# Thefefe/orbit

Hardware: AMD Instinct MI355X
Metric: meshlets_culled_per_sec (higher is better)
Workload: dtype f32

## Files before the change

### bindings/rust/orbit_hip.rs

```rust
#![allow(non_camel_case_types, dead_code)]
use std::ffi::{c_char, c_void};

#[repr(C)]
pub struct OrbitCtx { _private: [u8; 0] }
#[repr(C)]
pub struct OrbitMeshletStream { _private: [u8; 0] }

#[repr(C)] #[derive(Clone, Copy, Default)]
pub struct OrbitCaps {
    pub max_entities: u32, pub max_dispatches: u32, pub max_draws: u32, pub max_lights: u32,
    pub max_clusters: u32, pub dispatch_size: u32, pub max_views: u32, pub validate_streams: u32, pub cull_path: u32,
    pub arith_profile: u32,
}

#[repr(C)]
pub struct OrbitClusterFrame {
    pub push: *const c_void, pub info: *const c_void, pub depth: *const f32, pub lights: *const c_void,
    pub tile_depth_slice_mask: *mut u32, pub depth_bounds: *mut c_void, pub unique_cluster_buffer: *mut c_void,
    pub light_index_buffer: *mut c_void, pub cluster_offset_image: *mut u32,
    pub index_capacity: u32, pub light_index_capacity: u32,
}
#[repr(C)]
pub struct OrbitFrameLate {
    pub pyramids: *const c_void, pub late_views: *const c_void, pub cascade_views: *const c_void,
// ... 202 lines not shown
    pub fn orbit_meshlet_stream_set_materials(ctx: *mut OrbitCtx, ms: *mut OrbitMeshletStream, material_buffer: *const c_void,
                                              material_count: u32, stream: *mut c_void) -> i32;
    pub fn orbit_meshlet_stream_validate(ctx: *mut OrbitCtx, ms: *mut OrbitMeshletStream, meshlet_buffer: *const c_void,
                                         material_buffer: *const c_void, stream: *mut c_void) -> i32;
    pub fn orbit_meshlet_stream_destroy(ms: *mut OrbitMeshletStream) -> i32;
    pub fn orbit_meshlet_stream_update_meshes(ctx: *mut OrbitCtx, ms: *mut OrbitMeshletStream, mesh_info_buffer: *const c_void,
                                              first_mesh: u32, count: u32, stream: *mut c_void) -> i32;
    pub fn orbit_ctx_mesh_side_culls(ctx: *const OrbitCtx) -> u64;
    pub fn orbit_ctx_bind_meshlet_stream(ctx: *mut OrbitCtx, ms: *mut OrbitMeshletStream) -> i32;
    pub fn orbit_ctx_fused_culls(ctx: *const OrbitCtx) -> u64;
    pub fn orbit_frame_late(ctx: *mut OrbitCtx, frame: *const OrbitFrameLate, stream: *mut c_void) -> i32;
    pub fn orbit_ctx_meshlet_stream_culls(ctx: *const OrbitCtx) -> u64;
    pub fn orbit_ctx_meshlet_class_culls(ctx: *const OrbitCtx) -> u64;
    pub fn orbit_ctx_block_culls(ctx: *const OrbitCtx) -> u64;
    pub fn orbit_ctx_set_block_cull(ctx: *mut OrbitCtx, enable: u32) -> i32;
    pub fn orbit_meshlet_stream_block_bounds(ctx: *mut OrbitCtx, ms: *mut OrbitMeshletStream, first_block: u64, count: u64,
                                             out: *mut c_void, stream: *mut c_void) -> i32;
    pub fn orbit_p2p_alloc(ctx: *mut OrbitCtx, bytes: u64, out_ptr: *mut *mut c_void, out_handle: *mut [u8; 64]) -> i32;
    pub fn orbit_p2p_free(ctx: *mut OrbitCtx, ptr: *mut c_void) -> i32;
    pub fn orbit_p2p_open(ctx: *mut OrbitCtx, handle: *const [u8; 64], out_peer_ptr: *mut *mut c_void) -> i32;
    pub fn orbit_p2p_close(ctx: *mut OrbitCtx, peer_ptr: *mut c_void) -> i32;
    pub fn orbit_meshlet_cull_records_and_commands(ctx: *mut OrbitCtx, cull_info: *const c_void,
                                                   bufs: *const OrbitMeshletCullBufs, record_buffer: *mut c_void,
                                                   record_capacity: u32, stream: *mut c_void) -> i32;
    pub fn orbit_exchange_list(ctx: *mut OrbitCtx, local_list: *const c_void, rank: u32, world: u32,
                               out_buffers: *const *mut c_void, ctrl_buffers: *const *mut c_void, out_capacity: u32,
                               header_bytes: u32, stride: u32, stream: *mut c_void) -> i32;
    pub fn orbit_cull_shard(ctx: *mut OrbitCtx, cull_info: *const c_void, entity_bufs: *const OrbitEntityCullBufs,
                            draw_first: u32, draw_count: u32, meshlet_bufs: *const OrbitMeshletCullBufs,
                            record_buffer: *mut c_void, record_capacity: u32, with_commands: u32,
// ... 37 lines not shown
```

### include/orbit_abi_ext.h

```cpp
#ifndef ORBIT_ABI_EXT_H
#define ORBIT_ABI_EXT_H

#include "orbit_abi.h"

#ifdef __cplusplus
extern "C" {
#endif

#define ORBIT_VISIBLE_HEADER 8u
typedef struct OrbitVisibleRecord {
    uint32_t entity_index;
    uint32_t meshlet_offset;
    uint32_t mask;
} OrbitVisibleRecord;
ORBIT_STATIC_ASSERT(sizeof(OrbitVisibleRecord) == 12, "visible record is 12 B");

int32_t orbit_meshlet_task_cull(OrbitCtx *ctx, const OrbitGpuCullInfo *cull_info,
                                const OrbitMeshletCullBufs *bufs,
                                OrbitMeshTaskRecord *task_records, void *stream);

typedef struct OrbitCullView {
    const OrbitGpuCullInfo *cull_info;
    OrbitEntityCullBufs entity;
    OrbitMeshletCullBufs meshlet;
// ... 10 lines not shown
int32_t orbit_meshlet_stream_update(OrbitCtx *ctx, OrbitMeshletStream *ms, const void *meshlet_buffer,
                                    uint64_t first, uint64_t count, void *stream);
int32_t orbit_meshlet_stream_set_materials(OrbitCtx *ctx, OrbitMeshletStream *ms, const void *material_buffer,
                                           uint32_t material_count, void *stream);
int32_t orbit_meshlet_stream_validate(OrbitCtx *ctx, OrbitMeshletStream *ms, const void *meshlet_buffer,
                                      const void *material_buffer, void *stream);
int32_t orbit_meshlet_stream_update_meshes(OrbitCtx *ctx, OrbitMeshletStream *ms, const void *mesh_info_buffer,
                                           uint32_t first_mesh, uint32_t count, void *stream);
uint64_t orbit_ctx_mesh_side_culls(const OrbitCtx *ctx);
int32_t orbit_meshlet_stream_destroy(OrbitMeshletStream *ms);
int32_t orbit_ctx_bind_meshlet_stream(OrbitCtx *ctx, OrbitMeshletStream *ms);
uint64_t orbit_ctx_meshlet_stream_culls(const OrbitCtx *ctx);
uint64_t orbit_ctx_meshlet_class_culls(const OrbitCtx *ctx);
uint64_t orbit_ctx_block_culls(const OrbitCtx *ctx);
int32_t orbit_ctx_set_block_cull(OrbitCtx *ctx, uint32_t enable);
int32_t orbit_meshlet_stream_block_bounds(OrbitCtx *ctx, OrbitMeshletStream *ms, uint64_t first_block, uint64_t count,
                                          void *out, void *stream);

typedef struct OrbitDepthReduceItem {
    const float *depth;
    uint32_t screen_width, screen_height;
    uint32_t depth_row_pitch;
    uint32_t _pad;
    float *pyramid;
    const OrbitDepthPyramidLevel *levels;
} OrbitDepthReduceItem;
ORBIT_STATIC_ASSERT(sizeof(OrbitDepthReduceItem) == 40, "depth-reduce item is 40 B");
#define ORBIT_MAX_PYRAMID_BATCH 8
int32_t orbit_depth_reduce_multi(OrbitCtx *ctx, const OrbitDepthReduceItem *items, uint32_t count, void *stream);

// ... 268 lines not shown
```

### orbit_amd/_lib.py

```python
import ctypes as C
import os

_HERE = os.path.dirname(os.path.abspath(__file__))
LIB_PATH = os.path.join(_HERE, "liborbit_cull.so")

OK, E_INVALID, E_PLANES, E_CAPACITY, E_HIP, E_NO_DEVICE, E_TIMEOUT, E_MISSING, E_COMM, E_RANGE, E_STALE = (
    0, -1, -2, -3, -4, -5, -6, -7, -8, -9, -10)
ERROR_NAMES = {
    E_INVALID: "ORBIT_E_INVALID", E_PLANES: "ORBIT_E_PLANES", E_CAPACITY: "ORBIT_E_CAPACITY", E_HIP: "ORBIT_E_HIP",
    E_NO_DEVICE: "ORBIT_E_NO_DEVICE", E_TIMEOUT: "ORBIT_E_TIMEOUT", E_MISSING: "ORBIT_E_MISSING",
    E_COMM: "ORBIT_E_COMM", E_RANGE: "ORBIT_E_RANGE", E_STALE: "ORBIT_E_STALE",
}

MAX_PYRAMID_MIPS = 16


class OrbitError(RuntimeError):
    def __init__(self, code, message):
        super().__init__(f"{ERROR_NAMES.get(code, code)}: {message}")
        self.code = code


class Caps(C.Structure):
    _fields_ = [("max_entities", C.c_uint32), ("max_dispatches", C.c_uint32), ("max_draws", C.c_uint32),
# ... 144 lines not shown
    "orbit_p2p_open": (C.c_int32, [C.c_void_p, C.c_void_p, C.POINTER(C.c_void_p)]),
    "orbit_p2p_close": (C.c_int32, [C.c_void_p, C.c_void_p]),
    "orbit_meshlet_stream_create": (C.c_int32, [C.c_void_p, C.c_uint64, C.c_uint64, C.POINTER(C.c_void_p)]),
    "orbit_meshlet_stream_update": (C.c_int32, [C.c_void_p, C.c_void_p, C.c_void_p, C.c_uint64, C.c_uint64,
                                                C.c_void_p]),
    "orbit_meshlet_stream_set_materials": (C.c_int32, [C.c_void_p, C.c_void_p, C.c_void_p, C.c_uint32, C.c_void_p]),
    "orbit_meshlet_stream_validate": (C.c_int32, [C.c_void_p, C.c_void_p, C.c_void_p, C.c_void_p, C.c_void_p]),
    "orbit_meshlet_stream_destroy": (C.c_int32, [C.c_void_p]),
    "orbit_meshlet_stream_update_meshes": (C.c_int32, [C.c_void_p, C.c_void_p, C.c_void_p, C.c_uint32, C.c_uint32, C.c_void_p]),
    "orbit_ctx_mesh_side_culls": (C.c_uint64, [C.c_void_p]),
    "orbit_ctx_bind_meshlet_stream": (C.c_int32, [C.c_void_p, C.c_void_p]),
    "orbit_ctx_meshlet_stream_culls": (C.c_uint64, [C.c_void_p]),
    "orbit_ctx_meshlet_class_culls": (C.c_uint64, [C.c_void_p]),
    "orbit_ctx_block_culls": (C.c_uint64, [C.c_void_p]),
    "orbit_ctx_set_block_cull": (C.c_int32, [C.c_void_p, C.c_uint32]),
    "orbit_meshlet_stream_block_bounds": (C.c_int32, [C.c_void_p, C.c_void_p, C.c_uint64, C.c_uint64, C.c_void_p,
                                                      C.c_void_p]),
    "orbit_cull_shard": (C.c_int32, [C.c_void_p, C.c_void_p, C.POINTER(EntityCullBufs), C.c_uint32, C.c_uint32,
                                     C.POINTER(MeshletCullBufs), C.c_void_p, C.c_uint32, C.c_uint32, C.c_void_p]),
    "orbit_ctx_shard_culls": (C.c_uint64, [C.c_void_p]),
    "orbit_allgather_list": (C.c_int32, [C.c_void_p, C.c_void_p, C.c_uint32, C.c_uint32, C.c_void_p, C.c_uint32,
                                         C.c_void_p, C.c_void_p, C.c_uint32, C.c_uint32, C.c_uint32, C.c_void_p]),
    "orbit_compact_segments": (C.c_int32, [C.c_void_p, C.c_void_p, C.c_uint32, C.c_uint32, C.c_void_p, C.c_uint32,
                                           C.c_uint32, C.c_uint32, C.c_void_p]),
    "orbit_scene_update_entities": (C.c_int32, [C.c_void_p, C.c_void_p, C.c_void_p, C.c_uint32, C.c_void_p, C.c_uint32,
                                                C.c_void_p]),
    "orbit_scene_update": (C.c_int32, [C.c_void_p, C.POINTER(SceneUpdate), C.c_void_p]),
    "orbit_cull_stats": (C.c_int32, [C.c_void_p, C.c_void_p, C.POINTER(EntityCullBufs), C.c_uint32,
                                     C.POINTER(MeshletCullBufs), C.c_void_p, C.c_void_p]),
    "orbit_cluster_stats": (C.c_int32, [C.c_void_p, C.c_void_p, C.c_void_p, C.c_void_p, C.c_void_p, C.c_void_p,
# ... 49 lines not shown
```

### orbit_amd/csrc/abi_ctx.hip

```cpp
#include <cstdarg>
#include <cstdio>
#include <cstdlib>

#include "abi_internal.h"

thread_local char g_err[512] = "no error";

int32_t fail(OrbitCtx *ctx, int32_t code, const char *fmt, ...) {
    char buf[512];
    va_list ap;
    va_start(ap, fmt);
    vsnprintf(buf, sizeof(buf), fmt, ap);
    va_end(ap);
    snprintf(g_err, sizeof(g_err), "%s", buf);
    if (ctx) snprintf(ctx->err, sizeof(ctx->err), "%s", buf);
    return code;
}

namespace {

size_t layout_arena(OrbitCtx *ctx, uintptr_t base, uint64_t md32) {
    const OrbitCaps &caps = ctx->caps;
    const size_t ent = align_up((size_t)caps.max_entities, 256);
    const size_t mtiles = ((size_t)md32 + kTileRecords - 1) / kTileRecords + 1;
// ... 155 lines not shown
    if (!ctx) return ORBIT_OK;
    (void)hipSetDevice(ctx->device);
    (void)hipDeviceSynchronize();
    for (hipEvent_t ev : ctx->prof_events) (void)hipEventDestroy(ev);
    for (hipEvent_t ev : ctx->side_event)
        if (ev) (void)hipEventDestroy(ev);
    for (hipStream_t st : ctx->side_stream)
        if (st) (void)hipStreamDestroy(st);
    for (OrbitCtx *child : ctx->view_ctx) (void)orbit_ctx_destroy(child);
    if (ctx->meshlet_stream) ctx->meshlet_stream->bindings.fetch_sub(1);
    if (ctx->arena) (void)hipFree(ctx->arena);
    delete ctx;
    return ORBIT_OK;
}

int32_t orbit_ctx_status(OrbitCtx *ctx, void *stream, int32_t sync) {
    if (!ctx) return fail(nullptr, ORBIT_E_INVALID, "ctx is NULL");
    std::lock_guard<std::mutex> lock(ctx->mu);
    hipStream_t s = (hipStream_t)stream;
    if (sync) {
        hipError_t e = hipStreamSynchronize(s);
        if (e != hipSuccess) return hip_fail(ctx, e, "hipStreamSynchronize");
    }
    int32_t v = 0;
    hipError_t e = hipMemcpy(&v, ctx->status, 4, hipMemcpyDeviceToHost);
    if (e != hipSuccess) return hip_fail(ctx, e, "hipMemcpy(status)");
    for (OrbitCtx *child : ctx->view_ctx) {
        int32_t cv = 0;
        e = hipMemcpy(&cv, child->status, 4, hipMemcpyDeviceToHost);
        if (e != hipSuccess) return hip_fail(ctx, e, "hipMemcpy(status)");
// ... 124 lines not shown
```

### orbit_amd/csrc/abi_cull.hip

```cpp
#include "abi_internal.h"

namespace {

int32_t check_cull_info(OrbitCtx *ctx, const OrbitGpuCullInfo *ci) {
    if (!ci) return fail(ctx, ORBIT_E_INVALID, "cull_info is NULL");
    if (ci->cull_plane_count > ORBIT_MAX_CULL_PLANES)
        return fail(ctx, ORBIT_E_PLANES, "cull_plane_count %u > %d", ci->cull_plane_count, ORBIT_MAX_CULL_PLANES);
    if (ci->projection_type > 1) return fail(ctx, ORBIT_E_INVALID, "projection_type %u", ci->projection_type);
    if (ci->occlusion_pass > 2) return fail(ctx, ORBIT_E_INVALID, "occlusion_pass %u", ci->occlusion_pass);
    return ORBIT_OK;
}

MeshSideView mesh_side_for(OrbitMeshletStream *ms, const void *mesh_info_buffer, bool count = true) {
    if (!ms) return MeshSideView{nullptr, 0u};
    std::lock_guard<std::mutex> lock(ms->mu);
    if (ms->mesh_side == nullptr || ms->mesh_source != mesh_info_buffer || ms->mesh_hi == 0u) return MeshSideView{nullptr, 0u};
    if (count) ms->mesh_side_culls++;
    return MeshSideView{ms->mesh_side, ms->mesh_hi};
}

PyramidView make_pyramid_view(const float *texels, const uint32_t size[2],
                              const OrbitDepthPyramidLevel *levels = nullptr) {
    PyramidView v;
    v.texels = texels;
// ... 210 lines not shown
                          const MeshletCullOut &out, void *stream) {
    if (!ctx) return fail(nullptr, ORBIT_E_INVALID, "ctx is NULL");
    std::lock_guard<std::mutex> lock(ctx->mu);
    const hipStream_t s = (hipStream_t)stream;
    MeshletCullParams p;
    hipEvent_t ev0, ev1;
    int32_t rc = meshlet_cull_params(ctx, ctx, ci, b, out, p);
    if (rc == ORBIT_OK) rc = profile_pair(ctx, ev0, ev1);
    if (rc == ORBIT_OK && ci->occlusion_pass != 1) rc = validate_stream(ctx, p, s);
    if (rc) return rc;
    hipError_t e = hipSuccess;
    if (ctx->rec_shift > 5u) e = launch_split_records(split_params_for(ctx, ctx, b), s);
    if (e != hipSuccess) return hip_fail(ctx, e, "launch split_records");
    const bool blocks = ctx->block_cull && out.kind == MeshletCullOut::kCommands && p.ms.sphere != nullptr &&
                        p.ms.cls0 != nullptr && ci->occlusion_pass == 0u && ci->projection_type == 0u && p.arith == 0u;
    e = launch_meshlet_cull(p, ctx->num_cus, s, ev0, ev1, blocks ? stream_block_bounds(ctx->meshlet_stream) : nullptr);
    if (e != hipSuccess) return hip_fail(ctx, e, "launch meshlet_cull");
    count_stream_cull(ctx, p);
    if (blocks) ctx->block_culls++;
    return ORBIT_OK;
}

FusedCullParams fused_params(const EntityCullParams &ep, const MeshletCullParams &mp, const OrbitCtx *scratch,
                             uint32_t chunks) {
    FusedCullParams f{};
    f.m = mp;
    f.entity_draw_buffer = ep.entity_draw_buffer;
    f.mesh_infos = ep.mesh_infos;
    f.mesh_side = ep.mesh_side;
    f.visibility = ep.visibility;
    f.e_pyr = ep.pyr;
// ... 250 lines not shown
```

### orbit_amd/csrc/abi_internal.h

```cpp
#pragma once
#include <hip/hip_runtime.h>

#include <atomic>
#include <cstdint>
#include <cstring>
#include <mutex>
#include <new>
#include <vector>

#include "block_pretest.h"
#include "kernels.h"

using namespace orbit;

#pragma GCC visibility push(hidden)

struct OrbitMeshletStream {
    int device = 0;
    uint64_t first = 0, capacity = 0;
    uint4 *sphere = nullptr;
    uint32_t *cone = nullptr;
    uint16_t *mat = nullptr;
    uint32_t *cmd = nullptr;
    uint16_t *cnt = nullptr;
// ... 54 lines not shown
    uint32_t scan_patience = 256;
    unsigned long long *debug_cycles = nullptr;
    void *zero_page = nullptr;
    uint32_t profiling = 0;
    uint32_t prof_calls = 0;
    std::vector<hipEvent_t> prof_events;
    size_t prof_used = 0;
    std::vector<OrbitCtx *> view_ctx;
    hipStream_t side_stream[2] = {nullptr, nullptr};
    hipEvent_t side_event[3] = {nullptr, nullptr, nullptr};
    OrbitMeshletStream *meshlet_stream = nullptr;
    uint64_t stream_culls = 0;
    uint64_t class_culls = 0;
    uint64_t block_culls = 0;
    bool block_cull = true;
    char err[512] = {0};
};

constexpr uint32_t kExpandBlocks = 65536;

constexpr uint32_t kMeshBoundsSlots = 1024;

extern thread_local char g_err[512];

int32_t fail(OrbitCtx *ctx, int32_t code, const char *fmt, ...);

inline int32_t hip_fail(OrbitCtx *ctx, hipError_t e, const char *what) {
    return fail(ctx, ORBIT_E_HIP, "%s: %s", what, hipGetErrorString(e));
}

// ... 66 lines not shown
```

### orbit_amd/csrc/kernels.h

```cpp
#pragma once
#include <hip/hip_runtime.h>
#include <stdint.h>
#include <type_traits>

#include "../../include/orbit_abi_ext.h"
#include "orbit_device.h"

namespace orbit {

struct BlockBound;

constexpr uint32_t kTileRecords = 16;
constexpr uint32_t kTileRows = 8;
constexpr uint32_t kTicketPools = 8;
constexpr uint32_t kTicketStride = 64;
constexpr uint32_t kEmitTicketPools = 16;
constexpr uint32_t kListGroups = 32;
constexpr uint32_t kListSyncStride = 32;
constexpr uint32_t kListSyncWords = (kListGroups + 1) * kListSyncStride;

struct Payload {
    uint32_t y, z, w;
};

// ... 198 lines not shown
struct ViewGroup;
#if !ORBIT_CONTRACT
hipError_t launch_entity_cull_contracted(const EntityCullParams &p, uint32_t entity_draw_count, uint32_t num_cus, hipStream_t s);
hipError_t launch_entity_cull_views_contracted(const EntityCullViews &all, uint32_t n, uint32_t max_entity_draw_count,
                                               uint32_t num_cus, hipStream_t s);
hipError_t launch_meshlet_eval_contracted(const MeshletCullParams &p, uint32_t num_cus, hipStream_t s);
hipError_t launch_meshlet_eval_views_contracted(const MeshletCullViews &all, const ViewGroup &g, uint32_t m, uint32_t pass,
                                                bool ortho, int src, uint32_t max_tiles, uint32_t num_cus, hipStream_t s);
hipError_t launch_shard_cull_contracted(const FusedCullParams &f, uint32_t num_cus, hipStream_t s);
hipError_t launch_cull_fused_views_contracted(const FusedCullViews &all, const uint32_t *entity_draw_counts, uint32_t n,
                                              uint32_t num_cus, hipStream_t s);
#endif
hipError_t launch_entity_cull_views(const EntityCullViews &all, uint32_t n, uint32_t max_entity_draw_count,
                                    uint32_t num_cus, hipStream_t s);
hipError_t launch_meshlet_cull(const MeshletCullParams &p, uint32_t num_cus, hipStream_t s,
                               hipEvent_t ev0 = nullptr, hipEvent_t ev1 = nullptr, const BlockBound *blk = nullptr);
struct MeshletCullViews {
    MeshletCullParams v[ORBIT_MAX_CULL_VIEWS];
};
hipError_t launch_meshlet_cull_views(const MeshletCullViews &all, uint32_t n, uint32_t num_cus, hipStream_t s);
struct ViewGroup {
    uint8_t idx[ORBIT_MAX_CULL_VIEWS];
};
hipError_t launch_meshlet_eval(const MeshletCullParams &p, uint32_t num_cus, hipStream_t s);
hipError_t launch_meshlet_eval_blocks(const MeshletCullParams &p, const BlockBound *blk, dim3 grid, hipStream_t s);
uint32_t meshlet_eval_blocks_grid(uint32_t max_tiles, uint32_t num_cus);
hipError_t launch_meshlet_eval_views(const MeshletCullViews &all, const ViewGroup &g, uint32_t m, uint32_t pass,
                                     bool ortho, int src, uint32_t max_tiles, uint32_t num_cus, hipStream_t s);
hipError_t launch_meshlet_emit(const MeshletCullParams &p, bool stream, uint32_t num_cus, hipStream_t s);
hipError_t launch_meshlet_emit_views(const MeshletCullViews &all, const ViewGroup &g, uint32_t m, uint32_t n, bool stream,
                                     uint32_t max_tiles_all, uint32_t num_cus, hipStream_t s);
// ... 111 lines not shown
```

### orbit_amd/csrc/meshlet_cull.hip

```cpp
#include "kernels.h"

namespace orbit {

uint32_t max_dispatch_capacity() {
    const uint64_t cap = (uint64_t)kEmitChunkTable * kScanChunk * kTileRecords;
    return cap > 0xFFFFFFFFull ? 0xFFFFFFFFu : (uint32_t)cap;
}

namespace {

hipError_t scan_and_emit(const MeshletCullParams &p, uint32_t max_tiles, uint32_t num_cus, hipStream_t s) {
    const bool stream = p.ci.occlusion_pass != 1 && p.ms.sphere != nullptr;
    if (!stream) {
        const hipError_t e = launch_scan_chunks(p.tile_counts, p.tile_base, reinterpret_cast<const uint32_t *>(p.dispatch_buffer),
                                                kTileRecords, max_tiles, p.chunk_sums, s, p.tickets, kTicketPools * kTicketStride);
        if (e != hipSuccess) return e;
    }
    return launch_meshlet_emit(p, stream, num_cus, s);
}

}

hipError_t launch_meshlet_scan_emit(const MeshletCullParams &p, uint32_t num_cus, hipStream_t s) {
    const uint32_t max_tiles = (p.dispatch_capacity + kTileRecords - 1) / kTileRecords;
    if ((max_tiles + kScanChunk - 1) / kScanChunk > kEmitChunkTable) return hipErrorInvalidValue;
    return scan_and_emit(p, max_tiles, num_cus, s);
}

hipError_t launch_meshlet_cull(const MeshletCullParams &p, uint32_t num_cus, hipStream_t s, hipEvent_t ev0,
                               hipEvent_t ev1, const BlockBound *blk) {
    const uint32_t max_tiles = (p.dispatch_capacity + kTileRecords - 1) / kTileRecords;
    if ((max_tiles + kScanChunk - 1) / kScanChunk > kEmitChunkTable) return hipErrorInvalidValue;
    hipError_t e;
    if (ev0 && (e = hipEventRecord(ev0, s)) != hipSuccess) return e;
    if (blk != nullptr) {
        if (p.ci.occlusion_pass != 0u || p.ci.projection_type != 0u || p.arith != 0u || p.ms.cls0 == nullptr ||
            p.visible_list != 0u || p.task_records != nullptr)
            return hipErrorInvalidValue;
        e = launch_meshlet_eval_blocks(p, blk, dim3(meshlet_eval_blocks_grid(max_tiles, num_cus)), s);
    } else {
        e = launch_meshlet_eval(p, num_cus, s);
    }
    if (e != hipSuccess) return e;
    if (ev1 && (e = hipEventRecord(ev1, s)) != hipSuccess) return e;
    if (p.task_records) return launch_task_records(p, s);
    if (p.visible_list == 2u) {
        if (p.also_commands == nullptr) return hipSuccess;
        MeshletCullParams c = p;
        c.visible_list = 0u;
        c.draw_buffer = p.also_commands;
        c.draw_capacity = p.also_commands_capacity;
        return scan_and_emit(c, max_tiles, num_cus, s);
    }
    return scan_and_emit(p, max_tiles, num_cus, s);
// ... 56 lines not shown
```

### orbit_amd/csrc/meshlet_eval_blocks.hip

```cpp
#include "block_pretest.h"
#include "meshlet_common.h"

namespace orbit {

namespace {

constexpr int kBkWaves = 4;
constexpr int kBkWavesPerSimd = 5;
constexpr uint32_t kBkRing = 512, kBkFlush = 64;

struct __attribute__((aligned(16))) BlockTileLds {
    BlockRecord r[kTileRecords];
};
struct CandRing {
    uint16_t code[kBkRing];
};
struct RingState {
    uint32_t head = 0, count = 0;
    uint32_t total = 0;
};

__device__ __forceinline__ bool row_is_sparse(const WaveTileLds &L, int r) {
    const uint32_t w = reinterpret_cast<const uint32_t *>(&L.pad_)[0];
    return (((uint32_t)__builtin_amdgcn_readfirstlane((int)w) >> (2 * r)) & 1u) != 0u;
// ... 29 lines not shown
        const bool affine = ((aw >> (8 * ((lane >> 1) & 3))) & 1u) != 0u;
        BlockRecord o = block_record_setup(m, affine, R.scale, b, true, reinterpret_cast<const float *>(P.plane),
                                           min(p.ci.cull_plane_count, (uint32_t)ORBIT_MAX_CULL_PLANES));
        if (R.rec.z == 0u) o.flags = kBlkSparse;
        B.r[lane] = o;
        flags = o.flags;
    }
    uint64_t m = __ballot((flags & kBlkSparse) != 0u);
    m &= m >> 1;
    if (lane == 0) L.pad_ = m & 0x5555ull;
    __builtin_amdgcn_fence(__ATOMIC_RELEASE, "wavefront");
    __builtin_amdgcn_wave_barrier();
    __builtin_amdgcn_fence(__ATOMIC_ACQUIRE, "wavefront");
}

template <int R>
__device__ __forceinline__ void blk_row_load(const MeshletCullParams &p, const WaveTileLds &L, bool sparse, int lane,
                                             RowRegs<1> &t, const StreamRsrc &SR) {
    const uint32_t half = lane >> 5, ml = lane & 31;
    const uint4 rec = L.r[2 * R + half].rec;
    const bool active = ml < rec.z;
    const uint32_t rel = rec.y + ml - SR.first;
    const bool in = active & (rel < SR.count);
    if (active & !in) latch_status(p.status, ORBIT_E_RANGE);
    const uint32_t i = in ? rel : kNoOffset >> 4;
    const uint32_t is = sparse ? kNoOffset >> 4 : i;
    const auto sp = __builtin_amdgcn_raw_buffer_load_b128(SR.sphere, is << 4, 0, ORBIT_EVAL_LOAD_AUX);
    const uint32_t c = __builtin_amdgcn_raw_buffer_load_b32(SR.cone, i << 2, 0, ORBIT_EVAL_LOAD_AUX);
    t.a[0] = make_uint4(sp[0], sp[1], sp[2], sp[3]);
    t.b[0] = make_uint4(c, 0u, 0u, 0u);
    t.prev[0] = 0u;
}

template <int R>
__device__ __forceinline__ void blk_row_eval(WaveTileLds &L, const BlockTileLds &B, CandRing &ring, int lane,
                                             const RowRegs<1> &t, RingState &rs) {
    const uint32_t half = lane >> 5;
    const BlockRecord br = B.r[2 * R + half];
    float s0, band;
    block_pretest_terms(br, t.b[0].x, s0, band);
    const uint64_t culled = ballot(block_cone_culls(br, s0, band));
    const uint64_t kept = ballot(block_cone_keeps(s0, band)) & ballot((br.flags & kBlkInside) != 0u);
    const uint32_t lo = (uint32_t)__builtin_amdgcn_readfirstlane((int)L.r[2 * R].amask.x);
    const uint32_t hi = (uint32_t)__builtin_amdgcn_readfirstlane((int)L.r[2 * R + 1].amask.x);
    const uint64_t allow = (uint64_t)hi << 32 | lo;
    const uint64_t draw = allow & kept & ~culled;
    const uint64_t cand = allow & ~culled & ~kept;
    if (lane == 0) L.draw_mask[R] = draw;
    rs.total += (uint32_t)__popcll(draw);
    if (lane_of(cand)) ring.code[(rs.head + rs.count + lane_prefix(cand)) & (kBkRing - 1u)] = (uint16_t)(R * 64 + lane);
    rs.count += (uint32_t)__popcll(cand);
}

__device__ __forceinline__ void blk_flush(const MeshletCullParams &p, WaveTileLds &L, const PlaneLds &P, const CandRing &ring,
                                          const StreamRsrc &SR, int lane, RingState &rs, uint32_t n) {
// ... 12 lines not shown
    const uint64_t geo = eval_geometry_mask<0>(p, L, P, rid, make_uint4(sp[0], sp[1], sp[2], sp[3]), make_uint4(c, 0u, 0u, 0u), s, true);
    const uint64_t vis = geo & ballot(valid);
    if (lane_of(vis)) atomicOr(reinterpret_cast<uint32_t *>(L.draw_mask) + rid, 1u << ml);
    rs.total += (uint32_t)__popcll(vis);
    rs.head = (rs.head + n) & (kBkRing - 1u);
    rs.count -= n;
}

__global__ __launch_bounds__(kBkWaves * 64, kBkWavesPerSimd) void meshlet_eval_blocks_kernel(const MeshletCullParams p,
                                                                                            const BlockBound *blk) {
    __shared__ WaveTileLds lds[kBkWaves][3];
    __shared__ BlockTileLds blds[kBkWaves][2];
    __shared__ PlaneLds planes;
    __shared__ CandRing rings[kBkWaves];
    __shared__ uint32_t cls_sel[8];
    const int lane = threadIdx.x & 63, wave = threadIdx.x >> 6;
    const uint32_t nrec_raw = *reinterpret_cast<const uint32_t *>(p.dispatch_buffer);
    const uint32_t stride = gridDim.x * kBkWaves, wave_g = blockIdx.x * kBkWaves + wave;
    const uint32_t cap_tiles = (p.dispatch_capacity + kTileRecords - 1) / kTileRecords;
    uint4 r0 = setup_load_rec(p, wave_g, wave_g < cap_tiles, p.dispatch_capacity, lane);
    uint4 r1 = setup_load_rec(p, wave_g + stride, wave_g + stride < cap_tiles, p.dispatch_capacity, lane);
    uint4 rec2 = setup_load_rec(p, wave_g + 2u * stride, wave_g + 2u * stride < cap_tiles, p.dispatch_capacity, lane);
    planes_to_lds(p, planes);
    clear_chunk_sums(p, kBkWaves * 64);
    if (threadIdx.x < 6) cls_sel[threadIdx.x] = ((alpha_bits(p.ci, threadIdx.x >> 1) >> (threadIdx.x & 1u)) & 1u) ? ~0u : 0u;
    __syncthreads();
    const uint32_t nrec = min(nrec_raw, p.dispatch_capacity);
    const uint32_t ntiles = (nrec + kTileRecords - 1) / kTileRecords;
    const uint32_t full_rounds = ntiles / stride;
    const uint32_t dyn_rounds = min(max(full_rounds / 4u, 1u), 3u);
    const uint32_t n_static = ntiles <= stride ? 0xFFFFFFFFu : max(full_rounds >= dyn_rounds ? full_rounds - dyn_rounds : 0u, 3u);
    const uint32_t npools = min((uint32_t)kTicketPools, stride);
    const uint32_t pool = wave_g % npools;
// ... 14 lines not shown
        return t >= 0x08000000u ? 0xFFFFFFFFu : n_static * stride + t * npools + pool;
    };
    StreamRsrc SR = {};
    SR.first = p.ms.first;
    SR.count = p.ms.count;
    SR.sphere = __builtin_amdgcn_make_buffer_rsrc(const_cast<uint4 *>(p.ms.sphere + p.ms.first), 0, p.ms.count * 16u, kBufFlags);
    SR.cone = __builtin_amdgcn_make_buffer_rsrc(const_cast<uint32_t *>(p.ms.cone + p.ms.first), 0, p.ms.count * 4u, kBufFlags);
    uint32_t w0, w1, w2, tk_raw;
    {
        const uint32_t t0 = claim(), t1 = claim(), t2 = claim();
        tk_raw = claim();
        w0 = ticket_tile(t0, 0u);
        w1 = ticket_tile(t1, 1u);
        w2 = ticket_tile(t2, 2u);
    }
    RowRegs<1> qa, qb;
    {
        const uint4 none = make_uint4(0u, 0u, 0u, 0u);
        const uint32_t rl = (uint32_t)lane >> 2;
        if (!(w0 < ntiles && w0 * kTileRecords + rl < nrec)) r0 = none;
        if (!(w1 < ntiles && w1 * kTileRecords + rl < nrec)) r1 = none;
        if (!(w2 < ntiles && w2 * kTileRecords + rl < nrec)) rec2 = none;
        if ((lane & 3) == 0) lds[wave][0].r[lane >> 2].rec = r0;
        __builtin_amdgcn_fence(__ATOMIC_RELEASE, "wavefront");
        __builtin_amdgcn_wave_barrier();
        __builtin_amdgcn_fence(__ATOMIC_ACQUIRE, "wavefront");
        const float4 m0 = setup_load_mat(p, r0, lane);
        const float4 m1 = setup_load_mat(p, r1, lane);
        const uint32_t c0 = setup_load_cls(p, r0, lane), c1 = setup_load_cls(p, r1, lane);
        const BoundRegs b0 = blk_load_bound(p, blk, r0, lane), b1 = blk_load_bound(p, blk, r1, lane);
        blk_row_load<0>(p, lds[wave][0], false, lane, qa, SR);
        blk_row_load<1>(p, lds[wave][0], false, lane, qb, SR);
        setup_write_cls(lds[wave][0], cls_sel, r0, c0, lane);
        setup_write_cls(lds[wave][1], cls_sel, r1, c1, lane);
        setup_write(p, lds[wave][0], r0, m0, lane);
        blk_setup(p, lds[wave][0], blds[wave][0], planes, b0, lane);
        setup_write(p, lds[wave][1], r1, m1, lane);
        blk_setup(p, lds[wave][1], blds[wave][1], planes, b1, lane);
    }
    uint32_t it = 0;
    const uint32_t prio_rank = blockIdx.x / max(gridDim.x / (uint32_t)kBkWavesPerSimd, 1u);
    while (w0 < ntiles) {
        switch ((it + prio_rank) & 3u) {
        case 0: __builtin_amdgcn_s_setprio(0); break;
        case 1: __builtin_amdgcn_s_setprio(1); break;
        case 2: __builtin_amdgcn_s_setprio(2); break;
        default: __builtin_amdgcn_s_setprio(3); break;
        }
        const uint32_t w3 = ticket_tile(tk_raw, claims - 1u);
        tk_raw = claim();
        WaveTileLds &L = lds[wave][it % 3];
        WaveTileLds &Ln = lds[wave][(it + 1) % 3];
        const BlockTileLds &B = blds[wave][it & 1u];
        CandRing &ring = rings[wave];
        RingState rs;
#define BK_ROW(R, Q)                                                                                                   \
    if (row_is_sparse(L, R)) blk_row_eval<R>(L, B, ring, lane, Q, rs);                                                 \
    else rs.total = rows_eval<0, 0, R, 1, true>(p, L, planes, nullptr, lane, Q, rs.total, nullptr);
#define BK_FLUSH() \
    while (rs.count >= kBkFlush) blk_flush(p, L, planes, ring, SR, lane, rs, kBkFlush);
        BK_ROW(0, qa)
        blk_row_load<2>(p, L, row_is_sparse(L, 2), lane, qa, SR);
        BK_ROW(1, qb)
        blk_row_load<3>(p, L, row_is_sparse(L, 3), lane, qb, SR);
        BK_FLUSH()
        BK_ROW(2, qa)
        blk_row_load<4>(p, L, row_is_sparse(L, 4), lane, qa, SR);
        BK_ROW(3, qb)
        blk_row_load<5>(p, L, row_is_sparse(L, 5), lane, qb, SR);
        BK_FLUSH()
        const float4 mat2 = setup_load_mat(p, rec2, lane);
        const uint32_t cls2 = setup_load_cls(p, rec2, lane);
        const BoundRegs bnd2 = blk_load_bound(p, blk, rec2, lane);
        const uint4 rec3 = setup_load_rec(p, w3, w3 < ntiles, nrec, lane);
        BK_ROW(4, qa)
        blk_row_load<6>(p, L, row_is_sparse(L, 6), lane, qa, SR);
        BK_ROW(5, qb)
        blk_row_load<7>(p, L, row_is_sparse(L, 7), lane, qb, SR);
        BK_ROW(6, qa)
        blk_row_load<0>(p, Ln, row_is_sparse(Ln, 0), lane, qa, SR);
        BK_ROW(7, qb)
        blk_row_load<1>(p, Ln, row_is_sparse(Ln, 1), lane, qb, SR);
#undef BK_ROW
#undef BK_FLUSH
        setup_write_cls(lds[wave][(it + 2) % 3], cls_sel, rec2, cls2, lane);
        setup_write(p, lds[wave][(it + 2) % 3], rec2, mat2, lane);
        blk_setup(p, lds[wave][(it + 2) % 3], blds[wave][it & 1u], planes, bnd2, lane);
        while (rs.count > 0u) blk_flush(p, L, planes, ring, SR, lane, rs, min(rs.count, kBkFlush));
        __builtin_amdgcn_fence(__ATOMIC_RELEASE, "wavefront");
        __builtin_amdgcn_wave_barrier();
        __builtin_amdgcn_fence(__ATOMIC_ACQUIRE, "wavefront");
        if (lane < 2 * (int)kTileRows)
            p.tile_masks[(size_t)w0 * (2 * kTileRows) + lane] = reinterpret_cast<const uint32_t *>(L.draw_mask)[lane];
        if (lane == 0) p.tile_counts[w0] = rs.total;
        w0 = w1;
        w1 = w2;
        w2 = w3;
        rec2 = rec3;
        it++;
// ... 12 lines not shown
```

### orbit_amd/engine.py

```python
import ctypes as C

import numpy as np

from . import _lib, layouts


def _ptr(t):
    if t is None:
        return None
    if isinstance(t, int):
        return C.c_void_p(t)
    return C.c_void_p(t.data_ptr())


def _stream(stream):
    import torch

    s = torch.cuda.current_stream() if stream is None else stream
    return C.c_void_p(s.cuda_stream)


def _host_bytes(x, nbytes):
    a = np.ascontiguousarray(x).view(np.uint8).reshape(-1)
    if a.nbytes != nbytes:
# ... 516 lines not shown
    def fused_culls(self):
        return int(self._lib.orbit_ctx_fused_culls(self._ctx))

    def meshlet_stream_culls(self):
        return int(self._lib.orbit_ctx_meshlet_stream_culls(self._ctx))

    def meshlet_class_culls(self):
        return int(self._lib.orbit_ctx_meshlet_class_culls(self._ctx))

    def block_culls(self):
        return int(self._lib.orbit_ctx_block_culls(self._ctx))

    def set_block_cull(self, enable):
        _lib.check(self._lib.orbit_ctx_set_block_cull(self._ctx, 1 if enable else 0), self._ctx)

    def exchange_list(self, local_list, rank, world, out_buffers, ctrl_buffers, out_capacity, header_bytes, stride,
                      stream=None):
        outs = (C.c_void_p * world)(*[_ptr(b) for b in out_buffers])
        ctrls = (C.c_void_p * world)(*[_ptr(b) for b in ctrl_buffers])
        _lib.check(self._lib.orbit_exchange_list(self._ctx, _ptr(local_list), rank, world, outs, ctrls, out_capacity,
                                                 header_bytes, stride, _stream(stream)), self._ctx)

    def prepare_exchange_list(self, local_list, rank, world, out_buffers, ctrl_buffers, out_capacity, header_bytes, stride,
                              stream=None):
        outs = (C.c_void_p * world)(*[_ptr(b) for b in out_buffers])
        ctrls = (C.c_void_p * world)(*[_ptr(b) for b in ctrl_buffers])
        fn, ctx, lst, st = self._lib.orbit_exchange_list, self._ctx, _ptr(local_list), _stream(stream)
        keep = (outs, ctrls, local_list, stream)

        def call():
# ... 62 lines not shown
```

Before: 209.5 billion.

## Add whole-tile sparse fast path with full-tile cone prefetch in block cull

In the block-cull meshlet kernel, a tile whose LDS marker says every row is sparse now takes a fast path. All eight cone words are loaded up front, one per row, and the sphere loads are skipped. Next-tile prefetch is restructured to pick whole-tile or per-row loads, and wave indices are made scalar with readfirstlane. It also adds a context knob to cap the block-cull grid size, which defaults off. The aim is fewer wasted sphere loads and better latency hiding, at the cost of extra branching and register pressure.

```diff
diff --git a/bindings/rust/orbit_hip.rs b/bindings/rust/orbit_hip.rs
--- a/bindings/rust/orbit_hip.rs
+++ b/bindings/rust/orbit_hip.rs
@@ -240,6 +240,7 @@
     pub fn orbit_ctx_meshlet_class_culls(ctx: *const OrbitCtx) -> u64;
     pub fn orbit_ctx_block_culls(ctx: *const OrbitCtx) -> u64;
     pub fn orbit_ctx_set_block_cull(ctx: *mut OrbitCtx, enable: u32) -> i32;
+    pub fn orbit_ctx_set_block_cull_grid(ctx: *mut OrbitCtx, max_workgroups: u32) -> i32;
     pub fn orbit_meshlet_stream_block_bounds(ctx: *mut OrbitCtx, ms: *mut OrbitMeshletStream, first_block: u64, count: u64,
                                              out: *mut c_void, stream: *mut c_void) -> i32;
     pub fn orbit_p2p_alloc(ctx: *mut OrbitCtx, bytes: u64, out_ptr: *mut *mut c_void, out_handle: *mut [u8; 64]) -> i32;
diff --git a/include/orbit_abi_ext.h b/include/orbit_abi_ext.h
--- a/include/orbit_abi_ext.h
+++ b/include/orbit_abi_ext.h
@@ -48,6 +48,7 @@
 uint64_t orbit_ctx_meshlet_class_culls(const OrbitCtx *ctx);
 uint64_t orbit_ctx_block_culls(const OrbitCtx *ctx);
 int32_t orbit_ctx_set_block_cull(OrbitCtx *ctx, uint32_t enable);
+int32_t orbit_ctx_set_block_cull_grid(OrbitCtx *ctx, uint32_t max_workgroups);
 int32_t orbit_meshlet_stream_block_bounds(OrbitCtx *ctx, OrbitMeshletStream *ms, uint64_t first_block, uint64_t count,
                                           void *out, void *stream);
 
diff --git a/orbit_amd/_lib.py b/orbit_amd/_lib.py
--- a/orbit_amd/_lib.py
+++ b/orbit_amd/_lib.py
@@ -182,6 +182,7 @@
     "orbit_ctx_meshlet_class_culls": (C.c_uint64, [C.c_void_p]),
     "orbit_ctx_block_culls": (C.c_uint64, [C.c_void_p]),
     "orbit_ctx_set_block_cull": (C.c_int32, [C.c_void_p, C.c_uint32]),
+    "orbit_ctx_set_block_cull_grid": (C.c_int32, [C.c_void_p, C.c_uint32]),
     "orbit_meshlet_stream_block_bounds": (C.c_int32, [C.c_void_p, C.c_void_p, C.c_uint64, C.c_uint64, C.c_void_p,
                                                       C.c_void_p]),
     "orbit_cull_shard": (C.c_int32, [C.c_void_p, C.c_void_p, C.POINTER(EntityCullBufs), C.c_uint32, C.c_uint32,
diff --git a/orbit_amd/csrc/abi_ctx.hip b/orbit_amd/csrc/abi_ctx.hip
--- a/orbit_amd/csrc/abi_ctx.hip
+++ b/orbit_amd/csrc/abi_ctx.hip
@@ -193,6 +193,13 @@
     return ORBIT_OK;
 }
 
+int32_t orbit_ctx_set_block_cull_grid(OrbitCtx *ctx, uint32_t max_workgroups) {
+    if (!ctx) return fail(nullptr, ORBIT_E_INVALID, "ctx is NULL");
+    std::lock_guard<std::mutex> lock(ctx->mu);
+    ctx->block_cull_grid = max_workgroups;
+    return ORBIT_OK;
+}
+
 int32_t orbit_ctx_status(OrbitCtx *ctx, void *stream, int32_t sync) {
     if (!ctx) return fail(nullptr, ORBIT_E_INVALID, "ctx is NULL");
     std::lock_guard<std::mutex> lock(ctx->mu);
diff --git a/orbit_amd/csrc/abi_cull.hip b/orbit_amd/csrc/abi_cull.hip
--- a/orbit_amd/csrc/abi_cull.hip
+++ b/orbit_amd/csrc/abi_cull.hip
@@ -248,7 +248,8 @@
     if (e != hipSuccess) return hip_fail(ctx, e, "launch split_records");
     const bool blocks = ctx->block_cull && out.kind == MeshletCullOut::kCommands && p.ms.sphere != nullptr &&
                         p.ms.cls0 != nullptr && ci->occlusion_pass == 0u && ci->projection_type == 0u && p.arith == 0u;
-    e = launch_meshlet_cull(p, ctx->num_cus, s, ev0, ev1, blocks ? stream_block_bounds(ctx->meshlet_stream) : nullptr);
+    e = launch_meshlet_cull(p, ctx->num_cus, s, ev0, ev1, blocks ? stream_block_bounds(ctx->meshlet_stream) : nullptr,
+                            ctx->block_cull_grid);
     if (e != hipSuccess) return hip_fail(ctx, e, "launch meshlet_cull");
     count_stream_cull(ctx, p);
     if (blocks) ctx->block_culls++;
diff --git a/orbit_amd/csrc/abi_internal.h b/orbit_amd/csrc/abi_internal.h
--- a/orbit_amd/csrc/abi_internal.h
+++ b/orbit_amd/csrc/abi_internal.h
@@ -92,6 +92,7 @@
     uint64_t class_culls = 0;
     uint64_t block_culls = 0;
     bool block_cull = true;
+    uint32_t block_cull_grid = 0;
     char err[512] = {0};
 };
 
diff --git a/orbit_amd/csrc/kernels.h b/orbit_amd/csrc/kernels.h
--- a/orbit_amd/csrc/kernels.h
+++ b/orbit_amd/csrc/kernels.h
@@ -236,7 +236,8 @@
 hipError_t launch_entity_cull_views(const EntityCullViews &all, uint32_t n, uint32_t max_entity_draw_count,
                                     uint32_t num_cus, hipStream_t s);
 hipError_t launch_meshlet_cull(const MeshletCullParams &p, uint32_t num_cus, hipStream_t s,
-                               hipEvent_t ev0 = nullptr, hipEvent_t ev1 = nullptr, const BlockBound *blk = nullptr);
+                               hipEvent_t ev0 = nullptr, hipEvent_t ev1 = nullptr, const BlockBound *blk = nullptr,
+                               uint32_t blk_grid_cap = 0);
 struct MeshletCullViews {
     MeshletCullParams v[ORBIT_MAX_CULL_VIEWS];
 };
diff --git a/orbit_amd/csrc/meshlet_cull.hip b/orbit_amd/csrc/meshlet_cull.hip
--- a/orbit_amd/csrc/meshlet_cull.hip
+++ b/orbit_amd/csrc/meshlet_cull.hip
@@ -28,7 +28,7 @@
 }
 
 hipError_t launch_meshlet_cull(const MeshletCullParams &p, uint32_t num_cus, hipStream_t s, hipEvent_t ev0,
-                               hipEvent_t ev1, const BlockBound *blk) {
+                               hipEvent_t ev1, const BlockBound *blk, uint32_t blk_grid_cap) {
     const uint32_t max_tiles = (p.dispatch_capacity + kTileRecords - 1) / kTileRecords;
     if ((max_tiles + kScanChunk - 1) / kScanChunk > kEmitChunkTable) return hipErrorInvalidValue;
     hipError_t e;
@@ -37,7 +37,9 @@
         if (p.ci.occlusion_pass != 0u || p.ci.projection_type != 0u || p.arith != 0u || p.ms.cls0 == nullptr ||
             p.visible_list != 0u || p.task_records != nullptr)
             return hipErrorInvalidValue;
-        e = launch_meshlet_eval_blocks(p, blk, dim3(meshlet_eval_blocks_grid(max_tiles, num_cus)), s);
+        uint32_t grid = meshlet_eval_blocks_grid(max_tiles, num_cus);
+        if (blk_grid_cap != 0u) grid = min(grid, blk_grid_cap);
+        e = launch_meshlet_eval_blocks(p, blk, dim3(grid), s);
     } else {
         e = launch_meshlet_eval(p, num_cus, s);
     }
diff --git a/orbit_amd/csrc/meshlet_eval_blocks.hip b/orbit_amd/csrc/meshlet_eval_blocks.hip
--- a/orbit_amd/csrc/meshlet_eval_blocks.hip
+++ b/orbit_amd/csrc/meshlet_eval_blocks.hip
@@ -67,9 +67,18 @@
     __builtin_amdgcn_fence(__ATOMIC_ACQUIRE, "wavefront");
 }
 
+struct PipeRegs {
+    uint32_t v[10];
+};
+
+__device__ __forceinline__ bool tile_is_sparse(const WaveTileLds &L) {
+    const uint32_t w = reinterpret_cast<const uint32_t *>(&L.pad_)[0];
+    return (uint32_t)__builtin_amdgcn_readfirstlane((int)w) == 0x5555u;
+}
+
 template <int R>
 __device__ __forceinline__ void blk_row_load(const MeshletCullParams &p, const WaveTileLds &L, bool sparse, int lane,
-                                             RowRegs<1> &t, const StreamRsrc &SR) {
+                                             uint32_t *v, const StreamRsrc &SR) {
     const uint32_t half = lane >> 5, ml = lane & 31;
     const uint4 rec = L.r[2 * R + half].rec;
     const bool active = ml < rec.z;
@@ -79,19 +88,44 @@
     const uint32_t i = in ? rel : kNoOffset >> 4;
     const uint32_t is = sparse ? kNoOffset >> 4 : i;
     const auto sp = __builtin_amdgcn_raw_buffer_load_b128(SR.sphere, is << 4, 0, ORBIT_EVAL_LOAD_AUX);
-    const uint32_t c = __builtin_amdgcn_raw_buffer_load_b32(SR.cone, i << 2, 0, ORBIT_EVAL_LOAD_AUX);
-    t.a[0] = make_uint4(sp[0], sp[1], sp[2], sp[3]);
-    t.b[0] = make_uint4(c, 0u, 0u, 0u);
+    v[4] = __builtin_amdgcn_raw_buffer_load_b32(SR.cone, i << 2, 0, ORBIT_EVAL_LOAD_AUX);
+    v[0] = sp[0], v[1] = sp[1], v[2] = sp[2], v[3] = sp[3];
+}
+
+__device__ __forceinline__ void blk_tile_load(const MeshletCullParams &p, const WaveTileLds &L, int lane, uint32_t *v,
+                                              const StreamRsrc &SR) {
+    const uint32_t half = lane >> 5, ml = lane & 31;
+    bool bad = false;
+#pragma unroll
+    for (int r = 0; r < (int)kTileRows; r++) {
+        const uint4 rec = L.r[2 * r + half].rec;
+        const bool active = ml < rec.z;
+        const uint32_t rel = rec.y + ml - SR.first;
+        const bool in = active & (rel < SR.count);
+        bad |= active & !in;
+        const uint32_t i = in ? rel : kNoOffset >> 4;
+        v[r] = __builtin_amdgcn_raw_buffer_load_b32(SR.cone, i << 2, 0, ORBIT_EVAL_LOAD_AUX);
+    }
+    if (bad) latch_status(p.status, ORBIT_E_RANGE);
+}
+
+template <int R>
+__device__ __forceinline__ uint32_t blk_row_dense(const MeshletCullParams &p, WaveTileLds &L, const PlaneLds &P, int lane,
+                                                  const uint32_t *v, uint32_t total) {
+    RowRegs<1> t;
+    t.a[0] = make_uint4(v[0], v[1], v[2], v[3]);
+    t.b[0] = make_uint4(v[4], 0u, 0u, 0u);
     t.prev[0] = 0u;
+    return rows_eval<0, 0, R, 1, true>(p, L, P, nullptr, lane, t, total, nullptr);
 }
 
 template <int R>
 __device__ __forceinline__ void blk_row_eval(WaveTileLds &L, const BlockTileLds &B, CandRing &ring, int lane,
-                                             const RowRegs<1> &t, RingState &rs) {
+                                             uint32_t cone, RingState &rs) {
     const uint32_t half = lane >> 5;
     const BlockRecord br = B.r[2 * R + half];
     float s0, band;
-    block_pretest_terms(br, t.b[0].x, s0, band);
+    block_pretest_terms(br, cone, s0, band);
     const uint64_t culled = ballot(block_cone_culls(br, s0, band));
     const uint64_t kept = ballot(block_cone_keeps(s0, band)) & ballot((br.flags & kBlkInside) != 0u);
     const uint32_t lo = (uint32_t)__builtin_amdgcn_readfirstlane((int)L.r[2 * R].amask.x);
@@ -134,9 +168,9 @@
     __shared__ PlaneLds planes;
     __shared__ CandRing rings[kBkWaves];
     __shared__ uint32_t cls_sel[8];
-    const int lane = threadIdx.x & 63, wave = threadIdx.x >> 6;
+    const int lane = threadIdx.x & 63, wave = __builtin_amdgcn_readfirstlane((int)(threadIdx.x >> 6));
     const uint32_t nrec_raw = *reinterpret_cast<const uint32_t *>(p.dispatch_buffer);
-    const uint32_t stride = gridDim.x * kBkWaves, wave_g = blockIdx.x * kBkWaves + wave;
+    const uint32_t stride = gridDim.x * kBkWaves, wave_g = (uint32_t)__builtin_amdgcn_readfirstlane((int)(blockIdx.x * kBkWaves + wave));
     const uint32_t cap_tiles = (p.dispatch_capacity + kTileRecords - 1) / kTileRecords;
     uint4 r0 = setup_load_rec(p, wave_g, wave_g < cap_tiles, p.dispatch_capacity, lane);
     uint4 r1 = setup_load_rec(p, wave_g + stride, wave_g + stride < cap_tiles, p.dispatch_capacity, lane);
@@ -181,7 +215,9 @@
         w1 = ticket_tile(t1, 1u);
         w2 = ticket_tile(t2, 2u);
     }
-    RowRegs<1> qa, qb;
+    PipeRegs q;
+    bool whole;
+    uint32_t *const qa = q.v, *const qb = q.v + 5;
     {
         const uint4 none = make_uint4(0u, 0u, 0u, 0u);
         const uint32_t rl = (uint32_t)lane >> 2;
@@ -196,12 +232,18 @@
         const float4 m1 = setup_load_mat(p, r1, lane);
         const uint32_t c0 = setup_load_cls(p, r0, lane), c1 = setup_load_cls(p, r1, lane);
         const BoundRegs b0 = blk_load_bound(p, blk, r0, lane), b1 = blk_load_bound(p, blk, r1, lane);
-        blk_row_load<0>(p, lds[wave][0], false, lane, qa, SR);
-        blk_row_load<1>(p, lds[wave][0], false, lane, qb, SR);
         setup_write_cls(lds[wave][0], cls_sel, r0, c0, lane);
         setup_write_cls(lds[wave][1], cls_sel, r1, c1, lane);
         setup_write(p, lds[wave][0], r0, m0, lane);
         blk_setup(p, lds[wave][0], blds[wave][0], planes, b0, lane);
+        whole = tile_is_sparse(lds[wave][0]);
+        if (whole) {
+            blk_tile_load(p, lds[wave][0], lane, q.v, SR);
+            q.v[8] = q.v[9] = 0u;
+        } else {
+            blk_row_load<0>(p, lds[wave][0], row_is_sparse(lds[wave][0], 0), lane, qa, SR);
+            blk_row_load<1>(p, lds[wave][0], row_is_sparse(lds[wave][0], 1), lane, qb, SR);
+        }
         setup_write(p, lds[wave][1], r1, m1, lane);
         blk_setup(p, lds[wave][1], blds[wave][1], planes, b1, lane);
     }
@@ -221,35 +263,72 @@
         const BlockTileLds &B = blds[wave][it & 1u];
         CandRing &ring = rings[wave];
         RingState rs;
-#define BK_ROW(R, Q)                                                                                                   \
-    if (row_is_sparse(L, R)) blk_row_eval<R>(L, B, ring, lane, Q, rs);                                                 \
-    else rs.total = rows_eval<0, 0, R, 1, true>(p, L, planes, nullptr, lane, Q, rs.total, nullptr);
+        const bool nxt_whole = tile_is_sparse(Ln);
+        float4 mat2;
+        uint32_t cls2;
+        BoundRegs bnd2;
+        uint4 rec3;
 #define BK_FLUSH() \
     while (rs.count >= kBkFlush) blk_flush(p, L, planes, ring, SR, lane, rs, kBkFlush);
-        BK_ROW(0, qa)
-        blk_row_load<2>(p, L, row_is_sparse(L, 2), lane, qa, SR);
-        BK_ROW(1, qb)
-        blk_row_load<3>(p, L, row_is_sparse(L, 3), lane, qb, SR);
-        BK_FLUSH()
-        BK_ROW(2, qa)
-        blk_row_load<4>(p, L, row_is_sparse(L, 4), lane, qa, SR);
-        BK_ROW(3, qb)
-        blk_row_load<5>(p, L, row_is_sparse(L, 5), lane, qb, SR);
-        BK_FLUSH()
-        const float4 mat2 = setup_load_mat(p, rec2, lane);
-        const uint32_t cls2 = setup_load_cls(p, rec2, lane);
-        const BoundRegs bnd2 = blk_load_bound(p, blk, rec2, lane);
-        const uint4 rec3 = setup_load_rec(p, w3, w3 < ntiles, nrec, lane);
-        BK_ROW(4, qa)
-        blk_row_load<6>(p, L, row_is_sparse(L, 6), lane, qa, SR);
-        BK_ROW(5, qb)
-        blk_row_load<7>(p, L, row_is_sparse(L, 7), lane, qb, SR);
-        BK_ROW(6, qa)
-        blk_row_load<0>(p, Ln, row_is_sparse(Ln, 0), lane, qa, SR);
-        BK_ROW(7, qb)
-        blk_row_load<1>(p, Ln, row_is_sparse(Ln, 1), lane, qb, SR);
+        if (whole) {
+            PipeRegs tn;
+            if (nxt_whole) {
+                blk_tile_load(p, Ln, lane, tn.v, SR);
+                tn.v[8] = tn.v[9] = 0u;
+            } else {
+                blk_row_load<0>(p, Ln, row_is_sparse(Ln, 0), lane, tn.v, SR);
+                blk_row_load<1>(p, Ln, row_is_sparse(Ln, 1), lane, tn.v + 5, SR);
+            }
+            mat2 = setup_load_mat(p, rec2, lane);
+            cls2 = setup_load_cls(p, rec2, lane);
+            bnd2 = blk_load_bound(p, blk, rec2, lane);
+            rec3 = setup_load_rec(p, w3, w3 < ntiles, nrec, lane);
+            blk_row_eval<0>(L, B, ring, lane, q.v[0], rs);
+            blk_row_eval<1>(L, B, ring, lane, q.v[1], rs);
+            BK_FLUSH()
+            blk_row_eval<2>(L, B, ring, lane, q.v[2], rs);
+            blk_row_eval<3>(L, B, ring, lane, q.v[3], rs);
+            BK_FLUSH()
+            blk_row_eval<4>(L, B, ring, lane, q.v[4], rs);
+            blk_row_eval<5>(L, B, ring, lane, q.v[5], rs);
+            blk_row_eval<6>(L, B, ring, lane, q.v[6], rs);
+            blk_row_eval<7>(L, B, ring, lane, q.v[7], rs);
+            q = tn;
+        } else {
+#define BK_ROW(R, Q)                                                                                                   \
+    if (row_is_sparse(L, R)) blk_row_eval<R>(L, B, ring, lane, (Q)[4], rs);                                            \
+    else rs.total = blk_row_dense<R>(p, L, planes, lane, Q, rs.total);
+            BK_ROW(0, qa)
+            blk_row_load<2>(p, L, row_is_sparse(L, 2), lane, qa, SR);
+            BK_ROW(1, qb)
+            blk_row_load<3>(p, L, row_is_sparse(L, 3), lane, qb, SR);
+            BK_FLUSH()
+            BK_ROW(2, qa)
+            blk_row_load<4>(p, L, row_is_sparse(L, 4), lane, qa, SR);
+            BK_ROW(3, qb)
+            blk_row_load<5>(p, L, row_is_sparse(L, 5), lane, qb, SR);
+            BK_FLUSH()
+            mat2 = setup_load_mat(p, rec2, lane);
+            cls2 = setup_load_cls(p, rec2, lane);
+            bnd2 = blk_load_bound(p, blk, rec2, lane);
+            rec3 = setup_load_rec(p, w3, w3 < ntiles, nrec, lane);
+            BK_ROW(4, qa)
+            blk_row_load<6>(p, L, row_is_sparse(L, 6), lane, qa, SR);
+            BK_ROW(5, qb)
+            blk_row_load<7>(p, L, row_is_sparse(L, 7), lane, qb, SR);
+            BK_ROW(6, qa)
+            if (!nxt_whole) blk_row_load<0>(p, Ln, row_is_sparse(Ln, 0), lane, qa, SR);
+            BK_ROW(7, qb)
+            if (nxt_whole) {
+                blk_tile_load(p, Ln, lane, q.v, SR);
+                q.v[8] = q.v[9] = 0u;
+            } else {
+                blk_row_load<1>(p, Ln, row_is_sparse(Ln, 1), lane, qb, SR);
+            }
 #undef BK_ROW
+        }
 #undef BK_FLUSH
+        whole = nxt_whole;
         setup_write_cls(lds[wave][(it + 2) % 3], cls_sel, rec2, cls2, lane);
         setup_write(p, lds[wave][(it + 2) % 3], rec2, mat2, lane);
         blk_setup(p, lds[wave][(it + 2) % 3], blds[wave][it & 1u], planes, bnd2, lane);
diff --git a/orbit_amd/engine.py b/orbit_amd/engine.py
--- a/orbit_amd/engine.py
+++ b/orbit_amd/engine.py
@@ -554,6 +554,9 @@
     def set_block_cull(self, enable):
         _lib.check(self._lib.orbit_ctx_set_block_cull(self._ctx, 1 if enable else 0), self._ctx)
 
+    def set_block_cull_grid(self, max_workgroups):
+        _lib.check(self._lib.orbit_ctx_set_block_cull_grid(self._ctx, int(max_workgroups)), self._ctx)
+
     def exchange_list(self, local_list, rank, world, out_buffers, ctrl_buffers, out_capacity, header_bytes, stride,
                       stream=None):
         outs = (C.c_void_p * world)(*[_ptr(b) for b in out_buffers])
```

New measurement: 219.9 billion, median of 6. 5.0% higher.
